# xqtr/PySpecSDR

Measured on AMD Instinct MI355X. Metric: IQ MSamples/sec end-to-end (FFT+dB+FM demod), higher is better.
Workload: dtype complex64 IQ / f64 FFT + dB + post-process + FIR + IIR / dB rows stored as f32 / int16 PCM

## Files before the change

pyspecsdr_amd/csrc/pss_api.cpp:

```cpp
#include <hip/hip_runtime.h>

#include <cstdlib>
#include <cstring>
#include <string>
#include <vector>

#include "pss_ctx.h"

static std::string g_create_err;

int pss_fail(pss_ctx *ctx, int code, const std::string &msg)
{
    if (ctx) ctx->err = msg;
    else g_create_err = msg;
    return code;
}

int pss_hip_check(pss_ctx *ctx, hipError_t e, const char *what)
{
    if (e == hipSuccess) return PSS_OK;
    return pss_fail(ctx, PSS_E_HIP, std::string(what) + ": " + hipGetErrorString(e));
}

int pss_ensure_buffer(pss_ctx *ctx, void **buf, size_t *cap, size_t bytes, const char *what)
// ... 141 lines not shown
    }
    for (auto &kv : ctx->nfm) if (kv.second.d_rev) hipFree(kv.second.d_rev);
    if (ctx->scratch) hipFree(ctx->scratch);
    if (ctx->scratch_fft) hipFree(ctx->scratch_fft);
    if (ctx->scratch_hil) hipFree(ctx->scratch_hil);
    if (ctx->scratch_iqc) hipFree(ctx->scratch_iqc);
    if (ctx->d_hann) hipFree(ctx->d_hann);
    if (ctx->d_hann_short) hipFree(ctx->d_hann_short);
    ctx->st.release();
    if (ctx->scratch_scan) hipFree(ctx->scratch_scan);
    if (ctx->scratch_pk) hipFree(ctx->scratch_pk);
    if (ctx->scratch_win) hipFree(ctx->scratch_win);
    if (ctx->scratch_db64) hipFree(ctx->scratch_db64);
    if (ctx->scratch_post) hipFree(ctx->scratch_post);
    if (ctx->prog) hipFree(ctx->prog);
    if (ctx->stage) hipFree(ctx->stage);
    for (auto &b : ctx->sq_buf) if (b) hipFree(b);
    if (ctx->sq_pin) hipHostFree(ctx->sq_pin);
    for (PssDevTable *t : {&ctx->ddc_tab, &ctx->pfb_tab, &ctx->bank_tab, &ctx->rs_tab, &ctx->welch_win, &ctx->rds_tab, &ctx->rds_pulse, &ctx->ais_pulse}) t->release();
    if (ctx->welch_part) hipFree(ctx->welch_part);
    for (auto &b : ctx->adsb_buf) if (b) hipFree(b);
    if (ctx->adsb_pin) hipHostFree(ctx->adsb_pin);
    for (auto &b : ctx->ais_buf) if (b) hipFree(b);
    if (ctx->ais_pin) hipHostFree(ctx->ais_pin);
    hipEventDestroy(ctx->ev0);
    hipEventDestroy(ctx->ev1);
    hipStreamSynchronize(ctx->stream2);
    hipStreamDestroy(ctx->stream2);
    hipEventDestroy(ctx->ev_fork);
    hipEventDestroy(ctx->ev_join);
    if (ctx->ev_in) hipEventDestroy(ctx->ev_in);
    if (ctx->ev_out) hipEventDestroy(ctx->ev_out);
    for (auto &k : ctx->krecs) { hipEventDestroy(k.e0); hipEventDestroy(k.e1); }
    if (ctx->own_stream) hipStreamDestroy(ctx->stream);
    delete ctx;
}

extern "C" int pss_set_stream(pss_ctx *ctx, void *hip_stream)
{
    if (!ctx) return PSS_E_ARG;
    PSS_GUARD(ctx);
    hipStreamSynchronize(ctx->stream);
    if (ctx->own_stream) hipStreamDestroy(ctx->stream);
    ctx->stream = reinterpret_cast<hipStream_t>(hip_stream);
    ctx->own_stream = false;
    return PSS_OK;
}

extern "C" int pss_order_after(pss_ctx *ctx, void *hip_stream)
{
    if (!ctx) return PSS_E_ARG;
    PSS_GUARD(ctx);
    hipStream_t s = reinterpret_cast<hipStream_t>(hip_stream);
    if (s == ctx->stream) return PSS_OK;
    if (!ctx->ev_in) PSS_HIP(ctx, hipEventCreateWithFlags(&ctx->ev_in, hipEventDisableTiming));
    PSS_HIP(ctx, hipEventRecord(ctx->ev_in, s));
    PSS_HIP(ctx, hipStreamWaitEvent(ctx->stream, ctx->ev_in, 0));
    return PSS_OK;
}

extern "C" int pss_order_before(pss_ctx *ctx, void *hip_stream)
{
    if (!ctx) return PSS_E_ARG;
    PSS_GUARD(ctx);
    hipStream_t s = reinterpret_cast<hipStream_t>(hip_stream);
    if (s == ctx->stream) return PSS_OK;
    if (!ctx->ev_out) PSS_HIP(ctx, hipEventCreateWithFlags(&ctx->ev_out, hipEventDisableTiming));
    PSS_HIP(ctx, hipEventRecord(ctx->ev_out, ctx->stream));
    PSS_HIP(ctx, hipStreamWaitEvent(s, ctx->ev_out, 0));
    return PSS_OK;
}

extern "C" void *pss_get_stream(pss_ctx *ctx) { return ctx ? reinterpret_cast<void *>(ctx->stream) : nullptr; }

extern "C" int pss_set_option(pss_ctx *ctx, const char *key, int value)
{
    if (!ctx || !key) return PSS_E_ARG;
    if (!strcmp(key, "nfm_fused")) { ctx->no_fused = (value == 0); return PSS_OK; }
    if (!strcmp(key, "wfm_fused")) { ctx->no_wfm_fused = (value == 0); return PSS_OK; }
    if (!strcmp(key, "small_batch")) { ctx->no_small_batch = (value == 0); return PSS_OK; }
    if (!strcmp(key, "small_batch_max")) { ctx->small_batch_max = value; return PSS_OK; }
    if (!strcmp(key, "wfm_small_batch_max")) { ctx->wfm_small_batch_max = value; return PSS_OK; }
    if (!strcmp(key, "fuse_post")) { ctx->fuse_post = value != 0; return PSS_OK; }
    if (!strcmp(key, "ssb_rfft")) { ctx->ssb_rfft = value != 0; return PSS_OK; }
    if (!strcmp(key, "ssb_hilbert")) { ctx->ssb_hilbert = value != 0; return PSS_OK; }
    if (!strcmp(key, "hilbert_exact")) { ctx->hilbert_exact = value != 0; return PSS_OK; }
    if (!strcmp(key, "scan_exact")) { ctx->scan_exact = value != 0; return PSS_OK; }
    if (!strcmp(key, "db_exact")) { ctx->db_exact = value != 0; return PSS_OK; }
    if (!strcmp(key, "f64_plain")) { ctx->f64_plain = value != 0; return PSS_OK; }
    if (!strcmp(key, "wfm_corr_copy")) { ctx->wfm_corr_copy = value != 0; return PSS_OK; }
    return pss_fail(ctx, PSS_E_ARG, std::string("unknown option: ") + key);
}

extern "C" int pss_sync(pss_ctx *ctx)
{
    if (!ctx) return PSS_E_ARG;
    PSS_GUARD(ctx);
    return pss_hip_check(ctx, hipStreamSynchronize(ctx->stream), "hipStreamSynchronize");
}

extern "C" const char *pss_last_error(pss_ctx *ctx) { return ctx ? ctx->err.c_str() : g_create_err.c_str(); }

extern "C" int pss_enable_timing(pss_ctx *ctx, int on)
{
    if (!ctx) return PSS_E_ARG;
    PSS_GUARD(ctx);
    ctx->timing = on != 0;
    ctx->tdepth = 0;
    ctx->kused = 0;
    ctx->last_ms = -1.0f;
    return PSS_OK;
}

extern "C" int pss_timing_filter(pss_ctx *ctx, const char *kernel)
{
    if (!ctx) return PSS_E_ARG;
    PSS_GUARD(ctx);
    ctx->tfilter = kernel ? kernel : "";
    ctx->kused = 0;
    ctx->last_ms = -1.0f;
    return PSS_OK;
}

extern "C" float pss_last_kernel_ms(pss_ctx *ctx)
{
    if (!ctx || !ctx->timing || ctx->last_ms < 0.0f || !ctx->tfilter.empty()) return -1.0f;
    PSS_GUARD(ctx);
    if (hipEventSynchronize(ctx->ev1) != hipSuccess) return -1.0f;
    float ms = -1.0f;
    if (hipEventElapsedTime(&ms, ctx->ev0, ctx->ev1) != hipSuccess) return -1.0f;
    return ms;
}

extern "C" int pss_kernel_times(pss_ctx *ctx, char *buf, int buf_len)
{
    if (!ctx || !buf || buf_len < 1) return PSS_E_ARG;
    PSS_GUARD(ctx);
    std::string out;
    if (ctx->timing && ctx->last_ms >= 0.0f) {
        if (ctx->tfilter.empty()) hipEventSynchronize(ctx->ev1);
        else hipStreamSynchronize(ctx->stream);
        for (int i = 0; i < ctx->kused; i++) {
            float ms = 0.0f;
            if (hipEventElapsedTime(&ms, ctx->krecs[i].e0, ctx->krecs[i].e1) != hipSuccess) continue;
            out += ctx->krecs[i].name;
            out += "=" + std::to_string(ms) + ";";
        }
    }
    ctx->kused = 0;
    if ((int)out.size() + 1 > buf_len) return pss_fail(ctx, PSS_E_ARG, "buffer too small");
    memcpy(buf, out.c_str(), out.size() + 1);
    return PSS_OK;
}

namespace {
size_t up256(size_t x) { return (x + 255) & ~(size_t)255; }
}

extern "C" int pss_h_compute_fft(pss_ctx *ctx, const float *h_iq, int n, double *h_db)
{
    if (!ctx) return PSS_E_ARG;
    PSS_GUARD(ctx);
    if (!h_iq || !h_db || n < 1) return pss_fail(ctx, PSS_E_ARG, "bad arguments");
    const size_t o_db = up256(sizeof(float) * 2 * n);
    int r = pss_ensure_buffer(ctx, &ctx->stage, &ctx->stage_bytes, o_db + up256(sizeof(float) * n), "staging");
    if (r) return r;
// ... 295 lines not shown
```

pyspecsdr_amd/csrc/pss_ctx.h:

```cpp
#pragma once
#include <hip/hip_runtime.h>

#include <array>
#include <map>
#include <string>
#include <vector>

#include "../../include/pss.h"

struct PssNfmFilt {
    double taps[65];
    double sos[24];
    double zi[8];
    double *d_rev = nullptr;
};

struct PssWfmFilt {
    double lp[18], pilot[30], lmr[30];
    double alpha;
};

struct PssPairwisePlan {
    int n_leaves = 0, n_nodes = 0, n_levels = 0, n_roots = 0;
    int wave_tree = 0;
    int *d_tab = nullptr;
};

struct PssDevTable {
    void *dev = nullptr;
    size_t cap = 0;
    std::vector<unsigned char> host;
    void release()
    {
        if (dev) hipFree(dev);
        dev = nullptr, cap = 0;
        host.clear();
    }
};

struct PssStreaming {
    enum Slot {
        IQ = 0,
        DB = 2,
        PCM = 4,
        PLANE_A = 6,
        PLANE_B = 8,
        POST = 10,
        EXTREMES = 11,
        GRID_A = 12,
        GRID_B = 14,
        TAIL = 16,
        CODES = 18,
        NUMBERS = 20,
        WORK = 22,
        N_SLOTS
    };
    hipStream_t up = nullptr, dn = nullptr;
    hipEvent_t up_done[2] = {}, cmp_done[2] = {}, dn_done[2] = {};
    void *buf[N_SLOTS] = {};
    size_t cap[N_SLOTS] = {};
    int open(pss_ctx *ctx);
    int ensure(pss_ctx *ctx, int slot, size_t bytes, void **out);
    void release()
    {
        if (up) hipStreamDestroy(up);
        if (dn) hipStreamDestroy(dn);
        for (hipEvent_t *ev : {up_done, cmp_done, dn_done})
            for (int i = 0; i < 2; i++)
                if (ev[i]) hipEventDestroy(ev[i]);
        for (void *b : buf)
            if (b) hipFree(b);
        *this = PssStreaming{};
    }
};

struct pss_ctx {
    int device = 0;
    hipStream_t stream = nullptr;
    bool own_stream = false;
    hipStream_t stream2 = nullptr;
    hipStream_t cur = nullptr;
    hipEvent_t ev_fork = nullptr, ev_join = nullptr;
    hipEvent_t ev_in = nullptr, ev_out = nullptr;
    int n_cus = 0;
    int fuse_post = 1;
    double target_rate = 22050.0;
    bool wfm_corr_copy = false;
    std::string err;
    std::map<int, double2 *> tw;
    std::map<int, double *> win;
    std::map<int, double2 *> tw_pf;
    struct Bluestein { double2 *d_chirp; double2 *d_B; double *d_win; int M; };
    std::map<int, Bluestein> bs;
    std::map<double, PssNfmFilt> nfm;
    std::map<double, std::array<double, 65>> ssb;
    std::map<double, PssWfmFilt> wfm;
    std::map<int, PssPairwisePlan> plans;
    void *scratch = nullptr;
    size_t scratch_bytes = 0;
    void *scratch_iqc = nullptr;
    void *scratch_scan = nullptr;
    size_t scratch_scan_bytes = 0;
    void *scratch_pk = nullptr;
    size_t scratch_pk_bytes = 0;
    void *prog = nullptr;
    unsigned prog_epoch = 0;
    void *scratch_post = nullptr;
    size_t scratch_post_bytes = 0;
    void *scratch_db64 = nullptr;
    size_t scratch_db64_bytes = 0;
    void *scratch_win = nullptr;
    size_t scratch_win_bytes = 0;
    float *d_hann = nullptr;
    float hann_sum = 0.0f;
    PssStreaming st;
    float *d_hann_short = nullptr;
    float hann_short_sum = 0.0f;
    int hann_short_n = 0;
    size_t scratch_iqc_bytes = 0;
    void *scratch_fft = nullptr;
    size_t scratch_fft_bytes = 0;
    void *scratch_hil = nullptr;
    size_t scratch_hil_bytes = 0;
    void *stage = nullptr;
    size_t stage_bytes = 0;
    bool no_wfm_fused = false;
    long small_batch_max = 8192;
    long wfm_small_batch_max = 6000;
    bool hilbert_exact = false;
    bool ssb_rfft = true;
    bool ssb_hilbert = true;
    bool db_exact = false;
    bool f64_plain = false;
    bool scan_exact = true;
    bool no_small_batch = false;
    bool no_fused = false;
    void *comm = nullptr;
    int comm_rank = 0, comm_n = 1;
    void *sq_buf[3] = {};
    size_t sq_cap[3] = {};
    void *sq_pin = nullptr;
    PssDevTable ddc_tab;
    PssDevTable pfb_tab;
    PssDevTable bank_tab;
    PssDevTable rs_tab;
    PssDevTable welch_win;
    PssDevTable rds_tab;
    PssDevTable rds_pulse;
    void *adsb_buf[2] = {};
    size_t adsb_cap[2] = {};
    void *adsb_pin = nullptr;
    PssDevTable ais_pulse;
    void *ais_buf[2] = {};
    size_t ais_cap[2] = {};
    void *ais_pin = nullptr;
    void *welch_part = nullptr;
    size_t welch_part_bytes = 0;
    bool timing = false;
    std::string tfilter;
    bool kskip = false;
    int tdepth = 0;
    hipEvent_t ev0 = nullptr, ev1 = nullptr;
    float last_ms = -1.0f;
    struct KRec { const char *name; hipEvent_t e0, e1; };
    std::vector<KRec> krecs;
    int kused = 0;
};

// ... 28 lines not shown
int pss_fail(pss_ctx *ctx, int code, const std::string &msg);
int pss_hip_check(pss_ctx *ctx, hipError_t e, const char *what);
int pss_ensure_scratch(pss_ctx *ctx, size_t bytes);
int pss_ensure_buffer(pss_ctx *ctx, void **buf, size_t *cap, size_t bytes, const char *what);
int pss_table_sync(pss_ctx *ctx, PssDevTable *t, const void *img, size_t bytes, const char *what, size_t capacity = 0);
void pss_time_begin(pss_ctx *ctx);
void pss_time_end(pss_ctx *ctx);
struct PssTimeScope {
    pss_ctx *ctx;
    explicit PssTimeScope(pss_ctx *c) : ctx(c) { pss_time_begin(c); }
    ~PssTimeScope() { pss_time_end(ctx); }
    PssTimeScope(const PssTimeScope &) = delete;
    PssTimeScope &operator=(const PssTimeScope &) = delete;
};
void pss_kernel_begin(pss_ctx *ctx, const char *name);
void pss_kernel_end(pss_ctx *ctx);

#define PSS_STREAM(ctx) ((ctx)->cur ? (ctx)->cur : (ctx)->stream)

int pss_side_mark(pss_ctx *ctx);
int pss_side_wait(pss_ctx *ctx);
int pss_side_fork(pss_ctx *ctx);
int pss_side_join(pss_ctx *ctx);
template <class F>
int pss_on_side(pss_ctx *ctx, F &&f)
{
    PssStreamScope side(ctx->cur, ctx->stream2);
    return f();
}

struct PssIq {
    const float *f32 = nullptr;
    const double *f64 = nullptr;
};
struct PssBwdLaunch {
    const PssNfmFilt *flt = nullptr;
    bool stereo = false;
    double *Yf = nullptr, *Af = nullptr;
    int n = 0, q = 0, n_out = 0;
    long n_frames = 0;
    int16_t *d_pcm = nullptr; double *d_audio = nullptr;
    int launch(pss_ctx *ctx) const;
};
enum PssAfterFwd { PSS_RUN_ALL = 0, PSS_FORK_AFTER_FWD, PSS_DEFER_BWD };
struct PssDemodCall {
    bool correct = false;
    float *d_power = nullptr;
    PssAfterFwd after_fwd = PSS_RUN_ALL;
    bool forked = false;
    PssBwdLaunch bwd;
};
int pss_demod_run(pss_ctx *ctx, int mode, PssIq iq, long n_frames, int n, double fs, int16_t *d_pcm, double *d_audio, PssDemodCall *call);

#define PSS_HIP(ctx, call)                                         \
    do {                                                           \
        int _r = pss_hip_check((ctx), (call), #call);              \
        if (_r) return _r;                                         \
    } while (0)

int pss_iq_check(pss_ctx *ctx, int container, double scale, const float *h_table256);
struct PssIqFmt {
    bool codes = false;
    int container = 0;
    double scale = 0.0;
    const float *h_table256 = nullptr;
    static PssIqFmt of_codes(int container, double scale, const float *h_table256)
    {
        PssIqFmt f;
        f.codes = true, f.container = container, f.scale = scale, f.h_table256 = h_table256;
        return f;
    }
    size_t sample_bytes() const { return codes ? (size_t)pss_iq_code_bytes(container) : 2 * sizeof(float); }
};

int pss_gather_frames(pss_ctx *ctx, const float *d_iq, long n_frames, int n, const int32_t *d_idx, long n_idx, float *d_dst);

bool pss_hilbert_supported(int n);
int pss_hilbert_rows(pss_ctx *ctx, const double *d_x, long n_rows, int n, double *d_out, int out_mode, unsigned long long *d_maxbits,
                     int16_t *d_pcm);
int pss_fft_tables(pss_ctx *ctx, int n, const double2 **tw, const double **win);
bool pss_post_sel_serves(int n_fft, bool f64);
bool pss_spec_post_serves(const pss_ctx *ctx, int n_fft);
int pss_spec_post_chain(pss_ctx *ctx, const float *d_iq, long n_frames, int n_fft, float *d_db32, double *d_db64, double *d_lo, double *d_hi, int n_halo,
                        int window, int display, int disp_h, int disp_w, int8_t *d_a, int8_t *d_b, double *d_vals);
int pss_chain_vals_f32(pss_ctx *ctx, const float *d_db, long n_frames, int n_fft, float *d_lo, float *d_hi, int n_halo, int window, int display,
                       int disp_h, int disp_w, int8_t *d_a, int8_t *d_b, double *d_vals);
int pss_chain_vals_f64(pss_ctx *ctx, const double *d_db, long n_frames, int n_fft, double *d_lo, double *d_hi, int n_halo, int window, int display,
                       int disp_h, int disp_w, int8_t *d_a, int8_t *d_b, double *d_vals);
bool pss_ssb_fused_supported(int n);
float pss_h_atan2f_model(float y, float x);
double pss_np_tan(double x);
double pss_np_exp(double x);
int pss_design_firwin_kaiser(int numtaps, double cutoff, double beta, double *taps);
int pss_ssb_hilbert_fused(pss_ctx *ctx, const float *d_iq, long n_rows, int n, const double *taps65, double *d_audio, int16_t *d_pcm);
```

pyspecsdr_amd/csrc/pss_fft.hip:

```cpp
#include <hip/hip_runtime.h>

#include <cmath>
#include <vector>

#include "pss_ctx.h"
#include "pss_fft_r16.h"
#include "pss_fft_xl.h"
#include "pss_post.h"
#include "pss_bars.h"
#include "pss_views.h"
#include "pss_spec_post.h"
#include "pss_hilbert.h"
#include "pss_hilbert_pf.h"

namespace {

constexpr int TPB = 256;

inline int spec_flags(const pss_ctx *ctx) { return (ctx->scan_exact ? pss_r16::FLAG_SCAN_EXACT : 0) | (ctx->db_exact ? pss_r16::FLAG_DB_EXACT : 0); }
constexpr int LOG_NSUB_MAX = 12;
constexpr int STAGE_MAX_N = 16384;
constexpr int PT = 1024;

__device__ __forceinline__ double2 cmul(double2 a, double2 b)
// ... 1635 lines not shown
{
    if (!ctx) return PSS_E_ARG;
    PSS_GUARD(ctx);
    return row_extremes<float>(ctx, d_rows, n_rows, len, d_row_lo, d_row_hi);
}
extern "C" int pss_row_extremes_f64(pss_ctx *ctx, const double *d_rows, long n_rows, int len, double *d_row_lo, double *d_row_hi)
{
    if (!ctx) return PSS_E_ARG;
    PSS_GUARD(ctx);
    return row_extremes<double>(ctx, d_rows, n_rows, len, d_row_lo, d_row_hi);
}

extern "C" int pss_spectrum_post_f64(pss_ctx *ctx, const double *d_db, long n_frames, int n_fft, double *d_post, double *d_row_lo, double *d_row_hi)
{
    if (!ctx) return PSS_E_ARG;
    PSS_GUARD(ctx);
    if (n_frames < 0 || n_fft < 5 || (n_frames > 0 && (!d_db || !d_post))) return pss_fail(ctx, PSS_E_ARG, "pss_spectrum_post_f64: bad argument");
    if ((d_row_lo == nullptr) != (d_row_hi == nullptr)) return pss_fail(ctx, PSS_E_ARG, "pss_spectrum_post_f64: row_lo and row_hi go together");
    if (n_frames == 0) return PSS_OK;
    if (!ctx->f64_plain && n_fft >= 8 && post_sel_serves(n_fft, true)) {
        PssTimeScope timed(ctx);
        const int rq = post_sel_any<double>(ctx, d_db, n_frames, n_fft, d_post, d_row_lo, d_row_hi, nullptr, nullptr, 0);
        return rq;
    }
    PssTimeScope timed(ctx);
    pss_kernel_begin(ctx, "k_post_f64");
    hipLaunchKernelGGL(k_post_f64, dim3((unsigned)(n_frames < 2048 ? n_frames : 2048)), dim3(256), 0, PSS_STREAM(ctx), d_db, d_post, n_fft, n_frames);
    pss_kernel_end(ctx);
    int r = pss_hip_check(ctx, hipGetLastError(), "k_post_f64 launch");
    if (!r && d_row_lo) r = row_extremes<double>(ctx, d_post, n_frames, n_fft - 4, d_row_lo, d_row_hi);
    return r;
}

extern "C" int pss_spectrum_post_thresholds(pss_ctx *ctx, const float *d_db, long n_frames, int n_fft, float *d_row_thr, float *d_row_lo,
                                            float *d_row_hi)
{
    if (!ctx) return PSS_E_ARG;
    PSS_GUARD(ctx);
    if (n_frames > 0 && (!d_row_thr || !d_row_lo || !d_row_hi)) return pss_fail(ctx, PSS_E_ARG, "pss_spectrum_post_thresholds: null buffer");
    return spectrum_post(ctx, d_db, n_frames, n_fft, nullptr, d_row_lo, d_row_hi, d_row_thr);
}
extern "C" int pss_waterfall_rows_db(pss_ctx *ctx, const float *d_db, long n_frames, int n_fft, const float *d_row_thr, const float *d_row_lo,
                                     const float *d_row_hi, int n_halo, int window, int disp_w, int8_t *d_glyph, int8_t *d_colour)
{
    if (!ctx) return PSS_E_ARG;
    PSS_GUARD(ctx);
    if (n_frames > 0 && !d_row_thr) return pss_fail(ctx, PSS_E_ARG, "pss_waterfall_rows_db: null thresholds");
    return display_rows<float, 0>(ctx, d_db, n_frames, n_fft - 4, d_row_lo, d_row_hi, n_halo, window, 1, disp_w, d_glyph, d_colour, d_row_thr);
}
extern "C" int pss_persistence_rows_db(pss_ctx *ctx, const float *d_db, long n_frames, int n_fft, const float *d_row_thr,
                                       const float *d_row_lo, const float *d_row_hi, int n_halo, int window, int disp_h, int disp_w, int8_t *d_y)
{
    if (!ctx) return PSS_E_ARG;
    PSS_GUARD(ctx);
    if (n_frames > 0 && !d_row_thr) return pss_fail(ctx, PSS_E_ARG, "pss_persistence_rows_db: null thresholds");
    return display_rows<float, 1>(ctx, d_db, n_frames, n_fft - 4, d_row_lo, d_row_hi, n_halo, window, disp_h, disp_w, d_y, nullptr, d_row_thr);
}

bool pss_post_sel_serves(int n_fft, bool f64) { return n_fft >= 8 && post_sel_serves(n_fft, f64); }
template <class TR>
static int chain_vals(pss_ctx *ctx, const TR *d_db, long n_frames, int n_fft, TR *d_lo, TR *d_hi, int n_halo, int window, int display, int disp_h,
                      int disp_w, int8_t *d_a, int8_t *d_b, double *d_vals)
{
    if (n_frames == 0) return PSS_OK;
    PssTimeScope timed(ctx);
    int r = post_sel_any<TR>(ctx, d_db, n_frames, n_fft, (TR *)nullptr, d_lo + n_halo, d_hi + n_halo, (TR *)nullptr, d_vals, disp_w);
    if (!r) r = display == 2 ? display_rows<TR, 2>(ctx, (const TR *)nullptr, n_frames, n_fft - 4, d_lo, d_hi, n_halo, window, 1, disp_w, d_a, d_b, (const TR *)nullptr, d_vals)
              : display ? display_rows<TR, 1>(ctx, (const TR *)nullptr, n_frames, n_fft - 4, d_lo, d_hi, n_halo, window, disp_h, disp_w, d_a, nullptr, (const TR *)nullptr, d_vals)
                        : display_rows<TR, 0>(ctx, (const TR *)nullptr, n_frames, n_fft - 4, d_lo, d_hi, n_halo, window, 1, disp_w, d_a, d_b, (const TR *)nullptr, d_vals);
    return r;
}
int pss_chain_vals_f32(pss_ctx *ctx, const float *d_db, long n_frames, int n_fft, float *d_lo, float *d_hi, int n_halo, int window, int display,
                       int disp_h, int disp_w, int8_t *d_a, int8_t *d_b, double *d_vals)
{
    return chain_vals<float>(ctx, d_db, n_frames, n_fft, d_lo, d_hi, n_halo, window, display, disp_h, disp_w, d_a, d_b, d_vals);
}
int pss_chain_vals_f64(pss_ctx *ctx, const double *d_db, long n_frames, int n_fft, double *d_lo, double *d_hi, int n_halo, int window, int display,
                       int disp_h, int disp_w, int8_t *d_a, int8_t *d_b, double *d_vals)
{
    return chain_vals<double>(ctx, d_db, n_frames, n_fft, d_lo, d_hi, n_halo, window, display, disp_h, disp_w, d_a, d_b, d_vals);
}

bool pss_spec_post_serves(const pss_ctx *ctx, int n_fft) { return n_fft == 1024 && !ctx->f64_plain; }
int pss_spec_post_chain(pss_ctx *ctx, const float *d_iq, long n_frames, int n_fft, float *d_db32, double *d_db64, double *d_lo, double *d_hi,
                        int n_halo, int window, int display, int disp_h, int disp_w, int8_t *d_a, int8_t *d_b, double *d_vals)
{
    if (!pss_spec_post_serves(ctx, n_fft) || (!d_db32 && !d_db64)) return pss_fail(ctx, PSS_E_ARG, "fused transform + post-process: 1024-point frames, a row buffer");
    if (n_frames == 0) return PSS_OK;
    const double2 *tw;
    const double *win;
    int r = pss_fft_tables(ctx, n_fft, &tw, &win);
    if (r) return r;
    using C = pss_r16::Cfg<2>;
    auto kern = d_db32 ? (d_db64 ? pss_sp::k_spectrum_post<true, true> : pss_sp::k_spectrum_post<true, false>) : pss_sp::k_spectrum_post<false, true>;
    const size_t lds = (size_t)C::FPW * C::EX * sizeof(double2) + (size_t)C::TW2 * sizeof(double2);
    const long cap = 256L * 2 * 2;
    if (lds > 64 * 1024) PSS_HIP(ctx, hipFuncSetAttribute(reinterpret_cast<const void *>(kern), hipFuncAttributeMaxDynamicSharedMemorySize, (int)lds));
    const long groups = (n_frames + C::FPW - 1) / C::FPW;
    PssTimeScope timed(ctx);
    pss_kernel_begin(ctx, "k_spectrum_post");
    hipLaunchKernelGGL(kern, dim3((unsigned)(groups < cap ? groups : cap)), dim3(256), lds, PSS_STREAM(ctx), reinterpret_cast<const float2 *>(d_iq), d_db32,
                       d_db64, tw, win, n_frames, d_lo + n_halo, d_hi + n_halo, d_vals, disp_w);
    pss_kernel_end(ctx);
    r = pss_hip_check(ctx, hipGetLastError(), "k_spectrum_post launch");
    if (!r) r = display == 2 ? display_rows<double, 2>(ctx, (const double *)nullptr, n_frames, n_fft - 4, d_lo, d_hi, n_halo, window, 1, disp_w, d_a, d_b, (const double *)nullptr, d_vals)
              : display ? display_rows<double, 1>(ctx, (const double *)nullptr, n_frames, n_fft - 4, d_lo, d_hi, n_halo, window, disp_h, disp_w, d_a, nullptr, (const double *)nullptr, d_vals)
                        : display_rows<double, 0>(ctx, (const double *)nullptr, n_frames, n_fft - 4, d_lo, d_hi, n_halo, window, 1, disp_w, d_a, d_b, (const double *)nullptr, d_vals);
    return r;
}

extern "C" int pss_waterfall_rows(pss_ctx *ctx, const float *d_post, long n_frames, int len, const float *d_row_lo,
                                  const float *d_row_hi, int n_halo, int window, int disp_w, int8_t *d_glyph, int8_t *d_colour)
{
    if (!ctx) return PSS_E_ARG;
    PSS_GUARD(ctx);
    return display_rows<float, 0>(ctx, d_post, n_frames, len, d_row_lo, d_row_hi, n_halo, window, 1, disp_w, d_glyph, d_colour);
}
extern "C" int pss_waterfall_rows_f64(pss_ctx *ctx, const double *d_post, long n_frames, int len, const double *d_row_lo,
                                      const double *d_row_hi, int n_halo, int window, int disp_w, int8_t *d_glyph, int8_t *d_colour)
{
    if (!ctx) return PSS_E_ARG;
    PSS_GUARD(ctx);
    return display_rows<double, 0>(ctx, d_post, n_frames, len, d_row_lo, d_row_hi, n_halo, window, 1, disp_w, d_glyph, d_colour);
}
extern "C" int pss_gradient_rows(pss_ctx *ctx, const float *d_post, long n_frames, int len, const float *d_row_lo,
                                 const float *d_row_hi, int n_halo, int window, int disp_w, int8_t *d_glyph, int8_t *d_colour)
{
    if (!ctx) return PSS_E_ARG;
    PSS_GUARD(ctx);
    return display_rows<float, 2>(ctx, d_post, n_frames, len, d_row_lo, d_row_hi, n_halo, window, 1, disp_w, d_glyph, d_colour);
}
extern "C" int pss_gradient_rows_f64(pss_ctx *ctx, const double *d_post, long n_frames, int len, const double *d_row_lo,
                                     const double *d_row_hi, int n_halo, int window, int disp_w, int8_t *d_glyph, int8_t *d_colour)
{
    if (!ctx) return PSS_E_ARG;
    PSS_GUARD(ctx);
    return display_rows<double, 2>(ctx, d_post, n_frames, len, d_row_lo, d_row_hi, n_halo, window, 1, disp_w, d_glyph, d_colour);
}
extern "C" int pss_persistence_rows(pss_ctx *ctx, const float *d_post, long n_frames, int len, const float *d_row_lo,
                                    const float *d_row_hi, int n_halo, int window, int disp_h, int disp_w, int8_t *d_y)
{
    if (!ctx) return PSS_E_ARG;
    PSS_GUARD(ctx);
    return display_rows<float, 1>(ctx, d_post, n_frames, len, d_row_lo, d_row_hi, n_halo, window, disp_h, disp_w, d_y, nullptr);
}
extern "C" int pss_persistence_rows_f64(pss_ctx *ctx, const double *d_post, long n_frames, int len, const double *d_row_lo,
                                        const double *d_row_hi, int n_halo, int window, int disp_h, int disp_w, int8_t *d_y)
{
    if (!ctx) return PSS_E_ARG;
    PSS_GUARD(ctx);
    return display_rows<double, 1>(ctx, d_post, n_frames, len, d_row_lo, d_row_hi, n_halo, window, disp_h, disp_w, d_y, nullptr);
}

extern "C" int pss_waterfall_cells(pss_ctx *ctx, const float *d_rows, int n_rows, int len, int disp_h, int disp_w,
                                   int8_t *d_glyph, int8_t *d_colour)
{
    if (!ctx) return PSS_E_ARG;
    PSS_GUARD(ctx);
    if (!d_rows || !d_glyph || !d_colour || n_rows < 1 || len < 2 || disp_h < 1 || disp_w < 1)
        return pss_fail(ctx, PSS_E_ARG, "bad waterfall arguments");
    pss_kernel_begin(ctx, "k_cells");
    hipLaunchKernelGGL((k_cells<float, 0>), dim3(1), dim3(1024), 0, PSS_STREAM(ctx), d_rows, n_rows, len, disp_h, disp_w,
                       d_glyph, d_colour, 0, n_rows);
    pss_kernel_end(ctx);
    return pss_hip_check(ctx, hipGetLastError(), "k_cells launch");
}

extern "C" int pss_persistence_cells(pss_ctx *ctx, const float *d_rows, int n_rows, int len, int disp_h, int disp_w,
                                     int8_t *d_colour)
{
    if (!ctx) return PSS_E_ARG;
    PSS_GUARD(ctx);
    if (!d_rows || !d_colour || n_rows < 1 || len < 2 || disp_h < 1 || disp_w < 1)
        return pss_fail(ctx, PSS_E_ARG, "bad persistence arguments");
    pss_kernel_begin(ctx, "k_cells");
    hipLaunchKernelGGL((k_cells<float, 1>), dim3(1), dim3(1024), 0, PSS_STREAM(ctx), d_rows, n_rows, len, disp_h, disp_w,
                       (int8_t *)nullptr, d_colour, 0, n_rows);
    pss_kernel_end(ctx);
    return pss_hip_check(ctx, hipGetLastError(), "k_cells launch");
}

template <class T>
static int launch_spectrogram(pss_ctx *ctx, const T *d_rows, long n_rows, int len, int disp_h, int disp_w, int8_t *d_glyph,
                              int8_t *d_colour, double *d_range)
{
// ... 414 lines not shown
```

pyspecsdr_amd/csrc/pss_pipeline.hip:

```cpp
#include <hip/hip_runtime.h>

#include <string>

#include "pss_ctx.h"
#include "pss_rows.h"

extern "C" int pss_spectrum_nfm(pss_ctx *ctx, const float *d_iq, long n_frames, int n, double fs, float *d_db,
                                int16_t *d_pcm)
{
    if (!ctx) return PSS_E_ARG;
    PSS_GUARD(ctx);
    PssTimeScope timed(ctx);
    PssDemodCall call;
    call.after_fwd = PSS_FORK_AFTER_FWD;
    const int r2 = pss_demod_run(ctx, PSS_MODE_NFM, PssIq{d_iq}, n_frames, n, fs, d_pcm, nullptr, &call);
    int r;
    if (call.forked) {
        r = pss_side_wait(ctx);
        if (!r && !r2) r = pss_on_side(ctx, [&] { return pss_spectrum_db(ctx, d_iq, n_frames, n, d_db); });
        const int rj = pss_side_join(ctx);
        if (!r) r = rj;
    } else {
        r = r2 ? r2 : pss_spectrum_db(ctx, d_iq, n_frames, n, d_db);
    }
    return r2 ? r2 : r;
}

namespace {
template <class TR>
inline int pipe_lines(pss_ctx *ctx, int display, const TR *d_post, long nf, int len, const TR *lo, const TR *hi, int n_halo, int window, int disp_h,
                      int disp_w, int8_t *a, int8_t *b)
{
    return display == 2 ? pss_rows::gradient_rows(ctx, d_post, nf, len, lo, hi, n_halo, window, disp_w, a, b)
         : display ? pss_rows::persistence_rows(ctx, d_post, nf, len, lo, hi, n_halo, window, disp_h, disp_w, a)
                   : pss_rows::waterfall_rows(ctx, d_post, nf, len, lo, hi, n_halo, window, disp_w, a, b);
}
}

template <class TR>
static int frame_pipeline_impl(pss_ctx *ctx, int mode, const float *d_iq, long n_frames, int n, double fs, TR *d_db, TR *d_post,
                               TR *d_row_lo, TR *d_row_hi, int n_halo, int window, int display, int disp_h, int disp_w,
                               int8_t *d_glyph, int8_t *d_colour, int16_t *d_pcm, float *d_db32, bool demodulate);
template <class TR>
static int frame_pipeline(pss_ctx *ctx, int mode, const float *d_iq, long n_frames, int n, double fs, TR *d_db, TR *d_post,
                          TR *d_row_lo, TR *d_row_hi, int n_halo, int window, int display, int disp_h, int disp_w,
                          int8_t *d_glyph, int8_t *d_colour, int16_t *d_pcm, float *d_db32 = nullptr, bool demodulate = true)
{
    PssTimeScope timed(ctx);
    return frame_pipeline_impl<TR>(ctx, mode, d_iq, n_frames, n, fs, d_db, d_post, d_row_lo, d_row_hi, n_halo, window, display, disp_h, disp_w,
                                   d_glyph, d_colour, d_pcm, d_db32, demodulate);
}

__global__ __launch_bounds__(256) void k_rows_f64_to_f32(const double *__restrict__ src, float *__restrict__ dst, long count)
{
    for (long i = (long)blockIdx.x * blockDim.x + threadIdx.x; i < count; i += (long)gridDim.x * blockDim.x) dst[i] = (float)src[i];
}

template <class TR>
static int frame_pipeline_impl(pss_ctx *ctx, int mode, const float *d_iq, long n_frames, int n, double fs, TR *d_db, TR *d_post,
                               TR *d_row_lo, TR *d_row_hi, int n_halo, int window, int display, int disp_h, int disp_w,
                               int8_t *d_glyph, int8_t *d_colour, int16_t *d_pcm, float *d_db32, bool demodulate)
{
    constexpr bool F64 = sizeof(TR) == 8;
    if (n_frames < 0 || n_halo < 0 || window < 1 || disp_w < 1 || display < 0 || display > 2 || (display == 1 && (disp_h < 1 || disp_h > 127)))
        return pss_fail(ctx, PSS_E_ARG, "pss_frame_pipeline: bad frame count, halo, window or display geometry");
    if (n < 8) return pss_fail(ctx, PSS_E_ARG, "pss_frame_pipeline: frames of fewer than 8 samples have no post-processed row to draw");
    if (n_frames > 0 && (!d_iq || (!d_db && !d_db32) || !d_row_lo || !d_row_hi || !d_glyph || (!d_colour && display != 1) || (!d_pcm && demodulate)))
        return pss_fail(ctx, PSS_E_ARG, "pss_frame_pipeline: null buffer");
    double *d_vals = nullptr;
    if (n_frames > 0 && !d_post) {
        const bool direct = pss_post_sel_serves(n, F64) && !(F64 && ctx->f64_plain);
        const size_t need = direct ? (size_t)n_frames * disp_w * sizeof(double) : (size_t)n_frames * (n - 4) * sizeof(TR);
        int rq = pss_ensure_buffer(ctx, &ctx->scratch_post, &ctx->scratch_post_bytes, need, "post-process scratch");
        if (rq) return rq;
        if (direct) d_vals = reinterpret_cast<double *>(ctx->scratch_post);
        else d_post = reinterpret_cast<TR *>(ctx->scratch_post);
    }
    bool fused = false;
    if constexpr (F64) fused = ctx->fuse_post && d_vals && pss_spec_post_serves(ctx, n);
    if (n_frames > 0 && !d_db && !fused) {
        int rq = pss_ensure_buffer(ctx, &ctx->scratch_db64, &ctx->scratch_db64_bytes, (size_t)n_frames * n * sizeof(TR), "float64 dB rows");
        if (rq) return rq;
        d_db = reinterpret_cast<TR *>(ctx->scratch_db64);
    }
    auto spectrum_and_chain = [&]() -> int {
        if constexpr (F64) {
            if (fused)
                return pss_spec_post_chain(ctx, d_iq, n_frames, n, d_db32, d_db, d_row_lo, d_row_hi, n_halo, window, display, disp_h, disp_w, d_glyph,
                                           d_colour, d_vals);
        }
        int q = pss_rows::spectrum_db(ctx, d_iq, n_frames, n, d_db);
        if (q) return q;
        if (d_db32 && n_frames > 0) {
            const long count = n_frames * (long)n;
            pss_kernel_begin(ctx, "k_rows_f64_to_f32");
            hipLaunchKernelGGL(k_rows_f64_to_f32, dim3((unsigned)((count + 255) / 256 < 16384 ? (count + 255) / 256 : 16384)), dim3(256), 0, PSS_STREAM(ctx),
                               reinterpret_cast<const double *>(d_db), d_db32, count);
            pss_kernel_end(ctx);
            q = pss_hip_check(ctx, hipGetLastError(), "k_rows_f64_to_f32 launch");
            if (q) return q;
        }
        if (d_vals) return pss_rows::chain_vals(ctx, d_db, n_frames, n, d_row_lo, d_row_hi, n_halo, window, display, disp_h, disp_w, d_glyph, d_colour, d_vals);
        q = pss_rows::post(ctx, d_db, n_frames, n, d_post, d_row_lo + n_halo, d_row_hi + n_halo);
        if (!q) q = pipe_lines(ctx, display, d_post, n_frames, n - 4, d_row_lo, d_row_hi, n_halo, window, disp_h, disp_w, d_glyph, d_colour);
        return q;
    };
    if (!demodulate) return spectrum_and_chain();
    PssDemodCall call;
    call.correct = mode == PSS_MODE_WFM && n_frames > 0;
    PssTimeScope timed(ctx);
    if (mode != PSS_MODE_NFM && mode != PSS_MODE_WFM) {
        const int r = pss_side_fork(ctx);
        if (r) return r;
        const int rd = pss_demod_run(ctx, mode, PssIq{d_iq}, n_frames, n, fs, d_pcm, nullptr, &call);
        const int rc = pss_on_side(ctx, spectrum_and_chain);
        const int rj = pss_side_join(ctx);
        return rd ? rd : (rc ? rc : rj);
    }
    call.after_fwd = PSS_DEFER_BWD;
    int r = pss_demod_run(ctx, mode, PssIq{d_iq}, n_frames, n, fs, d_pcm, nullptr, &call);
    if (call.bwd.flt) {
        if (!r) r = pss_side_fork(ctx);
        if (!r) r = pss_on_side(ctx, spectrum_and_chain);
        const int rb = call.bwd.launch(ctx);
        const int rj = pss_side_join(ctx);
        if (!r) r = rb ? rb : rj;
    } else if (!r) {
        r = spectrum_and_chain();
    }
    return r;
}

extern "C" int pss_frame_pipeline_nfm_f64(pss_ctx *ctx, const float *d_iq, long n_frames, int n, double fs, double *d_db, double *d_post,
                                          double *d_row_lo, double *d_row_hi, int n_halo, int window, int disp_w, int8_t *d_glyph,
                                          int8_t *d_colour, int16_t *d_pcm)
{
    if (!ctx) return PSS_E_ARG;
    PSS_GUARD(ctx);
    if (n < 16 || n > 65536 || (n & (n - 1))) return pss_fail(ctx, PSS_E_ARG, "pss_frame_pipeline_nfm_f64: n must be a power of two in [16, 65536]");
    return frame_pipeline<double>(ctx, PSS_MODE_NFM, d_iq, n_frames, n, fs, d_db, d_post, d_row_lo, d_row_hi, n_halo, window, 0, 0, disp_w, d_glyph,
                                  d_colour, d_pcm);
}

extern "C" int pss_frame_pipeline_f64(pss_ctx *ctx, int mode, const float *d_iq, long n_frames, int n, double fs, double *d_db, double *d_post,
                                      double *d_row_lo, double *d_row_hi, int n_halo, int window, int display, int disp_h, int disp_w,
                                      int8_t *d_line_a, int8_t *d_line_b, int16_t *d_pcm)
{
    if (!ctx) return PSS_E_ARG;
    PSS_GUARD(ctx);
    if (mode < PSS_MODE_NFM || mode > PSS_MODE_WFM) return pss_fail(ctx, PSS_E_ARG, "unknown demodulation mode");
    if (n < 16 || n > 65536 || (n & (n - 1))) return pss_fail(ctx, PSS_E_ARG, "pss_frame_pipeline_f64: n must be a power of two in [16, 65536]");
    return frame_pipeline<double>(ctx, mode, d_iq, n_frames, n, fs, d_db, d_post, d_row_lo, d_row_hi, n_halo, window, display, disp_h, disp_w, d_line_a,
                                  d_line_b, d_pcm);
}

extern "C" int pss_frame_pipeline_cells(pss_ctx *ctx, int mode, const float *d_iq, long n_frames, int n, double fs, float *d_db32, double *d_db64,
                                        double *d_row_lo, double *d_row_hi, int n_halo, int window, int display, int disp_h, int disp_w, int8_t *d_line_a,
                                        int8_t *d_line_b, int16_t *d_pcm)
{
    if (!ctx) return PSS_E_ARG;
    PSS_GUARD(ctx);
    if (mode < PSS_MODE_NFM || mode > PSS_MODE_WFM) return pss_fail(ctx, PSS_E_ARG, "unknown demodulation mode");
    if (n < 16 || n > 65536 || (n & (n - 1))) return pss_fail(ctx, PSS_E_ARG, "pss_frame_pipeline_cells: n must be a power of two in [16, 65536]");
    if (n_frames > 0 && !d_db32) return pss_fail(ctx, PSS_E_ARG, "pss_frame_pipeline_cells: d_db32 is null");
    return frame_pipeline<double>(ctx, mode, d_iq, n_frames, n, fs, d_db64, nullptr, d_row_lo, d_row_hi, n_halo, window, display, disp_h, disp_w, d_line_a,
                                  d_line_b, d_pcm, d_db32);
}

extern "C" int pss_spectrum_cells(pss_ctx *ctx, const float *d_iq, long n_frames, int n, float *d_db32, double *d_db64, double *d_row_lo,
                                  double *d_row_hi, int n_halo, int window, int display, int disp_h, int disp_w, int8_t *d_line_a, int8_t *d_line_b)
{
    if (!ctx) return PSS_E_ARG;
    PSS_GUARD(ctx);
    if (n < 16 || n > 65536 || (n & (n - 1))) return pss_fail(ctx, PSS_E_ARG, "pss_spectrum_cells: n must be a power of two in [16, 65536]");
    if (n_frames > 0 && !d_db32 && !d_db64) return pss_fail(ctx, PSS_E_ARG, "pss_spectrum_cells: no row buffer");
    return frame_pipeline<double>(ctx, PSS_MODE_NFM, d_iq, n_frames, n, 0.0, d_db64, nullptr, d_row_lo, d_row_hi, n_halo, window, display, disp_h, disp_w,
                                  d_line_a, d_line_b, nullptr, d_db32, false);
}

template <class View>
static int view_pipeline(pss_ctx *ctx, const char *who, int mode, const float *d_iq, long n_frames, int n, double fs, float *d_db32, double *d_db64,
                         double *d_post, int16_t *d_pcm, View view)
{
    if (mode < PSS_MODE_NFM || mode > PSS_MODE_WFM) return pss_fail(ctx, PSS_E_ARG, "unknown demodulation mode");
    if (n < 16 || n > 65536 || (n & (n - 1))) return pss_fail(ctx, PSS_E_ARG, std::string(who) + ": n must be a power of two in [16, 65536]");
    if (n_frames > 0 && (!d_iq || !d_db32)) return pss_fail(ctx, PSS_E_ARG, std::string(who) + ": null buffer");
    if (n_frames == 0) return PSS_OK;
    if (!d_db64) {
        int rq = pss_ensure_buffer(ctx, &ctx->scratch_db64, &ctx->scratch_db64_bytes, (size_t)n_frames * n * sizeof(double), "float64 dB rows");
        if (rq) return rq;
        d_db64 = reinterpret_cast<double *>(ctx->scratch_db64);
    }
    if (!d_post) {
        int rq = pss_ensure_buffer(ctx, &ctx->scratch_post, &ctx->scratch_post_bytes, (size_t)n_frames * (n - 4) * sizeof(double), "post-process scratch");
        if (rq) return rq;
        d_post = reinterpret_cast<double *>(ctx->scratch_post);
    }
    auto display_chain = [&]() -> int {
        int q = pss_spectrum_db_f64(ctx, d_iq, n_frames, n, d_db64);
        if (q) return q;
        const long count = n_frames * (long)n;
        pss_kernel_begin(ctx, "k_rows_f64_to_f32");
        hipLaunchKernelGGL(k_rows_f64_to_f32, dim3((unsigned)((count + 255) / 256 < 16384 ? (count + 255) / 256 : 16384)), dim3(256), 0, PSS_STREAM(ctx),
                           d_db64, d_db32, count);
// ... 73 lines not shown
```

pyspecsdr_amd/csrc/pss_spec_post.h:

```cpp
#pragma once

namespace pss_sp {

using namespace pss_r16;

template <bool ROW32, bool ROW64>
__global__ __launch_bounds__(256, 2) void k_spectrum_post(const float2 *__restrict__ iq, float *__restrict__ db32, double *__restrict__ db64,
                                                       const double2 *__restrict__ tw, const double *__restrict__ win, long n_frames,
                                                       double *__restrict__ row_lo, double *__restrict__ row_hi, double *__restrict__ vals,
                                                       int disp_w)
{
    using C = Cfg<2>;
    constexpr int R3 = C::R3, T = C::T, N = C::N, FPW = C::FPW;
    static_assert(T == 64, "a frame is one wavefront");
    constexpr int EPL = 16;
    using PC = pss_post::PostCfg<EPL, double>;
    static_assert((size_t)(T + 1) * PC::S * sizeof(double) <= (size_t)C::EX * sizeof(double2), "the staged row fits the frame's exchange buffer");
    extern __shared__ __align__(16) unsigned char smem[];
    double2 *ex_all = reinterpret_cast<double2 *>(smem);
    double2 *tw2 = ex_all + (size_t)FPW * C::EX;
    const int tid = threadIdx.x;
    const int fl = __builtin_amdgcn_readfirstlane(tid / T);
    const int t = tid % T;
    double2 *ex = ex_all + (size_t)fl * C::EX;
    double *stage = reinterpret_cast<double *>(ex);
    double2 tw1[16];
    double w[16];
    tw1[0] = make_double2(1.0, 0.0);
#pragma unroll
    for (int k2 = 1; k2 < 16; k2++) tw1[k2] = tw[(size_t)t * k2];
#pragma unroll
    for (int n2 = 0; n2 < 16; n2++) w[n2] = win[t + T * n2];
    if (tid < R3 * 16) {
        const int m1 = tid / 16, j2 = tid % 16;
        tw2[C::tw2_slot(tid)] = tw[(size_t)(m1 * j2) * 16];
    }
    __syncthreads();
    const long groups = (n_frames + FPW - 1) / FPW;
    float2 nx[16];
    auto fetch = [&](long g) {
        const long f = g * FPW + fl;
        const float2 *x = iq + (size_t)(f < n_frames ? f : 0) * N;
#pragma unroll
        for (int n2 = 0; n2 < 16; n2++) nx[n2] = x[t + T * n2];
    };
    if ((long)blockIdx.x < groups) fetch(blockIdx.x);
    int phase = 0;
    for (long g = blockIdx.x; g < groups; g += gridDim.x) {
        const long f = g * FPW + fl;
        const bool valid = f < n_frames;
        double2 v[16];
#pragma unroll
        for (int n2 = 0; n2 < 16; n2++) v[n2] = make_double2((double)nx[n2].x * w[n2], (double)nx[n2].y * w[n2]);
        if (g + gridDim.x < groups) fetch(g + gridDim.x);
        const long f_first = g * FPW;
        const long rows_here = n_frames - f_first < FPW ? n_frames - f_first : FPW;
        const __amdgpu_buffer_rsrc_t ro32 = make_rsrc((ROW32 && db32) ? db32 + (size_t)f_first * N : nullptr, (ROW32 && db32) ? (unsigned)(rows_here * N * 4) : 0u);
        const __amdgpu_buffer_rsrc_t ro64 = make_rsrc((ROW64 && db64) ? db64 + (size_t)f_first * N : nullptr, (ROW64 && db64) ? (unsigned)(rows_here * N * 8) : 0u);
        const int lane_el = fl * N + t;
        double dbv[16];
        unsigned hmax = 0;
        auto emit = [&](int i, int, double2 X) {
            const double pw = power_of(X);
            hmax = max(hmax, db_hi32(pw));
            dbv[i] = db64_core(pw);
        };
        r16_core<2, true>(v, ex, tw1, tw2, t, emit);
        if (__builtin_amdgcn_ballot_w64(hmax >= DB_HI_NONFINITE) != 0) {
#pragma unroll
            for (int i = 0; i < 16; i++) {
                const double d = dbv[i];
                const double nonfinite = d == DB_NONFINITE_IMAGE ? __builtin_inf() : __builtin_copysign(__builtin_nan(""), d);
                dbv[i] = __builtin_fabs(d) < DB_FINITE_LIMIT ? d : nonfinite;
            }
        }
#pragma unroll
        for (int i = 0; i < 16; i++) {
            const int e0 = ((256 * (i % R3) + T * (i / R3)) + N / 2) & (N - 1);
            if constexpr (ROW64) buf_store_f64(ro64, lane_el * 8, e0 * 8, dbv[i]);
            if constexpr (ROW32) buf_store_f32(ro32, lane_el * 4, e0 * 4, (float)dbv[i]);
        }
        frame_sync<true>();
#pragma unroll
        for (int i = 0; i < 16; i++) {
            const int c = i / R3, j1 = i % R3;
            const int e = (((256 * j1 + T * c) + N / 2) & (N - 1)) + t;
            stage[(e / EPL) * PC::S + (e % EPL)] = dbv[i];
        }
        frame_sync<true>();
        if (valid) {
            int slot[PC::Q];
#pragma unroll
            for (int j = 0; j < PC::Q; j++) slot[j] = 0;
            pss_post::post_row_staged<EPL, 1, true, double>(stage, slot, t, N - 4, nullptr, fl, t, phase, nullptr, row_lo, row_hi, f, nullptr, vals, disp_w);
        }
        frame_sync<true>();
    }
}

}
```

Before: 70270.

## Partition fused spectrum-post work unevenly across workgroups to balance beside concurrent demod

Replaces the grid-stride loop in the fused FFT+dB+post kernel with contiguous per-workgroup ranges. The first n_cus workgroups get d extra groups, with d sized from the concurrent backward-demod launch (NFM vs WFM), so the workgroups that share compute units with the side-stream demod kernel finish at about the same time. It also caps the grid at 2*n_cus instead of a fixed 1024 and adds an optional timestamp probe under a compile flag. The risks are that the heuristic split may mismatch how the hardware actually places workgroups, and that contiguous ranges change the memory access order.

```diff
diff --git a/pyspecsdr_amd/csrc/pss_api.cpp b/pyspecsdr_amd/csrc/pss_api.cpp
--- a/pyspecsdr_amd/csrc/pss_api.cpp
+++ b/pyspecsdr_amd/csrc/pss_api.cpp
@@ -247,6 +247,7 @@
     if (!strcmp(key, "small_batch_max")) { ctx->small_batch_max = value; return PSS_OK; }
     if (!strcmp(key, "wfm_small_batch_max")) { ctx->wfm_small_batch_max = value; return PSS_OK; }
     if (!strcmp(key, "fuse_post")) { ctx->fuse_post = value != 0; return PSS_OK; }
+    if (!strcmp(key, "post_split")) { ctx->post_split = value < 0 ? -1 : value; return PSS_OK; }
     if (!strcmp(key, "ssb_rfft")) { ctx->ssb_rfft = value != 0; return PSS_OK; }
     if (!strcmp(key, "ssb_hilbert")) { ctx->ssb_hilbert = value != 0; return PSS_OK; }
     if (!strcmp(key, "hilbert_exact")) { ctx->hilbert_exact = value != 0; return PSS_OK; }
diff --git a/pyspecsdr_amd/csrc/pss_ctx.h b/pyspecsdr_amd/csrc/pss_ctx.h
--- a/pyspecsdr_amd/csrc/pss_ctx.h
+++ b/pyspecsdr_amd/csrc/pss_ctx.h
@@ -84,6 +84,7 @@
     hipEvent_t ev_in = nullptr, ev_out = nullptr;
     int n_cus = 0;
     int fuse_post = 1;
+    int post_split = -1;
     double target_rate = 22050.0;
     bool wfm_corr_copy = false;
     std::string err;
@@ -278,7 +279,7 @@
 bool pss_post_sel_serves(int n_fft, bool f64);
 bool pss_spec_post_serves(const pss_ctx *ctx, int n_fft);
 int pss_spec_post_chain(pss_ctx *ctx, const float *d_iq, long n_frames, int n_fft, float *d_db32, double *d_db64, double *d_lo, double *d_hi, int n_halo,
-                        int window, int display, int disp_h, int disp_w, int8_t *d_a, int8_t *d_b, double *d_vals);
+                        int window, int display, int disp_h, int disp_w, int8_t *d_a, int8_t *d_b, double *d_vals, const PssBwdLaunch *beside_bwd = nullptr);
 int pss_chain_vals_f32(pss_ctx *ctx, const float *d_db, long n_frames, int n_fft, float *d_lo, float *d_hi, int n_halo, int window, int display,
                        int disp_h, int disp_w, int8_t *d_a, int8_t *d_b, double *d_vals);
 int pss_chain_vals_f64(pss_ctx *ctx, const double *d_db, long n_frames, int n_fft, double *d_lo, double *d_hi, int n_halo, int window, int display,
diff --git a/pyspecsdr_amd/csrc/pss_fft.hip b/pyspecsdr_amd/csrc/pss_fft.hip
--- a/pyspecsdr_amd/csrc/pss_fft.hip
+++ b/pyspecsdr_amd/csrc/pss_fft.hip
@@ -1741,8 +1741,19 @@
 }
 
 bool pss_spec_post_serves(const pss_ctx *ctx, int n_fft) { return n_fft == 1024 && !ctx->f64_plain; }
+#ifdef PSS_EXP_POST_STAMPS
+static unsigned long long *g_post_stamps = nullptr;
+static long g_post_stamps_wg = 0;
+extern "C" long pss_exp_post_stamps(unsigned long long *h_out, long max_wg)
+{
+    if (!g_post_stamps || hipDeviceSynchronize() != hipSuccess) return -1;
+    const long n = g_post_stamps_wg < max_wg ? g_post_stamps_wg : max_wg;
+    return hipMemcpy(h_out, g_post_stamps, (size_t)n * 2 * sizeof(unsigned long long), hipMemcpyDeviceToHost) == hipSuccess ? n : -1;
+}
+#endif
 int pss_spec_post_chain(pss_ctx *ctx, const float *d_iq, long n_frames, int n_fft, float *d_db32, double *d_db64, double *d_lo, double *d_hi,
-                        int n_halo, int window, int display, int disp_h, int disp_w, int8_t *d_a, int8_t *d_b, double *d_vals)
+                        int n_halo, int window, int display, int disp_h, int disp_w, int8_t *d_a, int8_t *d_b, double *d_vals,
+                        const PssBwdLaunch *beside_bwd)
 {
     if (!pss_spec_post_serves(ctx, n_fft) || (!d_db32 && !d_db64)) return pss_fail(ctx, PSS_E_ARG, "fused transform + post-process: 1024-point frames, a row buffer");
     if (n_frames == 0) return PSS_OK;
@@ -1753,13 +1764,38 @@
     using C = pss_r16::Cfg<2>;
     auto kern = d_db32 ? (d_db64 ? pss_sp::k_spectrum_post<true, true> : pss_sp::k_spectrum_post<true, false>) : pss_sp::k_spectrum_post<false, true>;
     const size_t lds = (size_t)C::FPW * C::EX * sizeof(double2) + (size_t)C::TW2 * sizeof(double2);
-    const long cap = 256L * 2 * 2;
+    const long ncu = ctx->n_cus > 0 ? ctx->n_cus : 256;
+    const long cap = ncu * 2;
     if (lds > 64 * 1024) PSS_HIP(ctx, hipFuncSetAttribute(reinterpret_cast<const void *>(kern), hipFuncAttributeMaxDynamicSharedMemorySize, (int)lds));
     const long groups = (n_frames + C::FPW - 1) / C::FPW;
+    const long n_wg = groups < cap ? groups : cap;
+    constexpr long PSS_POST_SPLIT_D_NFM = 16, PSS_POST_SPLIT_D_WFM = 0;
+    long d = 0;
+    if (ctx->post_split >= 0) {
+        d = ctx->post_split;
+    } else if (beside_bwd && beside_bwd->flt) {
+        const long simds = ncu * 4;
+        const long bwd_waves = ((beside_bwd->n_frames + 63) / 64) * (beside_bwd->stereo ? 2 : 1);
+        d = (beside_bwd->stereo ? PSS_POST_SPLIT_D_WFM : PSS_POST_SPLIT_D_NFM) * (3 * simds + 2 * (bwd_waves < simds ? bwd_waves : simds)) / (5 * simds);
+    }
+    const PssPostSplit split = pss_post_split_shares(groups, n_wg, ncu, d);
+#ifdef PSS_EXP_POST_STAMPS
+    if (g_post_stamps_wg < n_wg) {
+        if (g_post_stamps) PSS_HIP(ctx, hipFree(g_post_stamps));
+        g_post_stamps = nullptr, g_post_stamps_wg = 0;
+        PSS_HIP(ctx, hipMalloc(&g_post_stamps, (size_t)cap * 2 * sizeof(unsigned long long)));
+        g_post_stamps_wg = cap;
+    }
+#endif
     PssTimeScope timed(ctx);
     pss_kernel_begin(ctx, "k_spectrum_post");
-    hipLaunchKernelGGL(kern, dim3((unsigned)(groups < cap ? groups : cap)), dim3(256), lds, PSS_STREAM(ctx), reinterpret_cast<const float2 *>(d_iq), d_db32,
-                       d_db64, tw, win, n_frames, d_lo + n_halo, d_hi + n_halo, d_vals, disp_w);
+#ifdef PSS_EXP_POST_STAMPS
+    hipLaunchKernelGGL(kern, dim3((unsigned)n_wg), dim3(256), lds, PSS_STREAM(ctx), reinterpret_cast<const float2 *>(d_iq), d_db32,
+                       d_db64, tw, win, n_frames, d_lo + n_halo, d_hi + n_halo, d_vals, disp_w, split.n_early, split.share_early, split.share_late, g_post_stamps);
+#else
+    hipLaunchKernelGGL(kern, dim3((unsigned)n_wg), dim3(256), lds, PSS_STREAM(ctx), reinterpret_cast<const float2 *>(d_iq), d_db32,
+                       d_db64, tw, win, n_frames, d_lo + n_halo, d_hi + n_halo, d_vals, disp_w, split.n_early, split.share_early, split.share_late);
+#endif
     pss_kernel_end(ctx);
     r = pss_hip_check(ctx, hipGetLastError(), "k_spectrum_post launch");
     if (!r) r = display == 2 ? display_rows<double, 2>(ctx, (const double *)nullptr, n_frames, n_fft - 4, d_lo, d_hi, n_halo, window, 1, disp_w, d_a, d_b, (const double *)nullptr, d_vals)
diff --git a/pyspecsdr_amd/csrc/pss_pipeline.hip b/pyspecsdr_amd/csrc/pss_pipeline.hip
--- a/pyspecsdr_amd/csrc/pss_pipeline.hip
+++ b/pyspecsdr_amd/csrc/pss_pipeline.hip
@@ -83,11 +83,12 @@
         if (rq) return rq;
         d_db = reinterpret_cast<TR *>(ctx->scratch_db64);
     }
+    const PssBwdLaunch *beside_bwd = nullptr;
     auto spectrum_and_chain = [&]() -> int {
         if constexpr (F64) {
             if (fused)
                 return pss_spec_post_chain(ctx, d_iq, n_frames, n, d_db32, d_db, d_row_lo, d_row_hi, n_halo, window, display, disp_h, disp_w, d_glyph,
-                                           d_colour, d_vals);
+                                           d_colour, d_vals, beside_bwd);
         }
         int q = pss_rows::spectrum_db(ctx, d_iq, n_frames, n, d_db);
         if (q) return q;
@@ -120,6 +121,7 @@
     call.after_fwd = PSS_DEFER_BWD;
     int r = pss_demod_run(ctx, mode, PssIq{d_iq}, n_frames, n, fs, d_pcm, nullptr, &call);
     if (call.bwd.flt) {
+        beside_bwd = &call.bwd;
         if (!r) r = pss_side_fork(ctx);
         if (!r) r = pss_on_side(ctx, spectrum_and_chain);
         const int rb = call.bwd.launch(ctx);
diff --git a/pyspecsdr_amd/csrc/pss_post_split.h b/pyspecsdr_amd/csrc/pss_post_split.h
--- /dev/null
+++ b/pyspecsdr_amd/csrc/pss_post_split.h
@@ -0,0 +1,44 @@
+#pragma once
+
+#if defined(__HIPCC__)
+#define PSS_SPLIT_HD __host__ __device__
+#else
+#define PSS_SPLIT_HD
+#endif
+
+struct PssPostSplit {
+    long n_early;
+    long share_early;
+    long share_late;
+};
+
+PSS_SPLIT_HD inline PssPostSplit pss_post_split_shares(long groups, long n_wg, long n_early, long d)
+{
+    PssPostSplit s;
+    s.n_early = n_early < 0 ? 0 : (n_early > n_wg ? n_wg : n_early);
+    if (d < 0 || s.n_early == 0 || s.n_early == n_wg) d = 0;
+    if (groups < n_wg) {
+        s.share_early = s.share_late = 1;
+        return s;
+    }
+    if (d > 0 && n_wg + s.n_early * d > groups) d = (groups - n_wg) / s.n_early;
+    s.share_late = (groups - s.n_early * d) / n_wg;
+    s.share_early = s.share_late + d;
+    return s;
+}
+
+PSS_SPLIT_HD inline void pss_post_split_range(long groups, long n_wg, long n_early, long share_early, long share_late, long b, long *begin, long *end)
+{
+    const long covered = n_early * share_early + (n_wg - n_early) * share_late;
+    const long left = groups > covered ? groups - covered : 0;
+    const long first_extra = n_wg - left;
+    long g0 = b < n_early ? b * share_early : n_early * share_early + (b - n_early) * share_late;
+    long len = b < n_early ? share_early : share_late;
+    if (b > first_extra) g0 += b - first_extra;
+    if (b >= first_extra) len += 1;
+    long g1 = g0 + len;
+    if (g0 > groups) g0 = groups;
+    if (g1 > groups) g1 = groups;
+    *begin = g0;
+    *end = g1;
+}
diff --git a/pyspecsdr_amd/csrc/pss_spec_post.h b/pyspecsdr_amd/csrc/pss_spec_post.h
--- a/pyspecsdr_amd/csrc/pss_spec_post.h
+++ b/pyspecsdr_amd/csrc/pss_spec_post.h
@@ -1,4 +1,6 @@
 #pragma once
+
+#include "pss_post_split.h"
 
 namespace pss_sp {
 
@@ -8,8 +10,15 @@
 __global__ __launch_bounds__(256, 2) void k_spectrum_post(const float2 *__restrict__ iq, float *__restrict__ db32, double *__restrict__ db64,
                                                        const double2 *__restrict__ tw, const double *__restrict__ win, long n_frames,
                                                        double *__restrict__ row_lo, double *__restrict__ row_hi, double *__restrict__ vals,
-                                                       int disp_w)
+                                                       int disp_w, long n_early, long share_early, long share_late
+#ifdef PSS_EXP_POST_STAMPS
+                                                       , unsigned long long *__restrict__ stamps
+#endif
+)
 {
+#ifdef PSS_EXP_POST_STAMPS
+    if (threadIdx.x == 0) stamps[2 * (size_t)blockIdx.x] = wall_clock64();
+#endif
     using C = Cfg<2>;
     constexpr int R3 = C::R3, T = C::T, N = C::N, FPW = C::FPW;
     static_assert(T == 64, "a frame is one wavefront");
@@ -44,15 +53,17 @@
 #pragma unroll
         for (int n2 = 0; n2 < 16; n2++) nx[n2] = x[t + T * n2];
     };
-    if ((long)blockIdx.x < groups) fetch(blockIdx.x);
+    long g_first, g_end;
+    pss_post_split_range(groups, (long)gridDim.x, n_early, share_early, share_late, (long)blockIdx.x, &g_first, &g_end);
+    if (g_first < g_end) fetch(g_first);
     int phase = 0;
-    for (long g = blockIdx.x; g < groups; g += gridDim.x) {
+    for (long g = g_first; g < g_end; g++) {
         const long f = g * FPW + fl;
         const bool valid = f < n_frames;
         double2 v[16];
 #pragma unroll
         for (int n2 = 0; n2 < 16; n2++) v[n2] = make_double2((double)nx[n2].x * w[n2], (double)nx[n2].y * w[n2]);
-        if (g + gridDim.x < groups) fetch(g + gridDim.x);
+        if (g + 1 < g_end) fetch(g + 1);
         const long f_first = g * FPW;
         const long rows_here = n_frames - f_first < FPW ? n_frames - f_first : FPW;
         const __amdgpu_buffer_rsrc_t ro32 = make_rsrc((ROW32 && db32) ? db32 + (size_t)f_first * N : nullptr, (ROW32 && db32) ? (unsigned)(rows_here * N * 4) : 0u);
@@ -96,6 +107,9 @@
         }
         frame_sync<true>();
     }
+#ifdef PSS_EXP_POST_STAMPS
+    if (threadIdx.x == 0) stamps[2 * (size_t)blockIdx.x + 1] = wall_clock64();
+#endif
 }
 
 }
```

After: 71180, median of 6. 1.3% higher.
